# Clemapfel/egg_fluid_simulation

Measured on AMD Instinct MI355X. Metric: pair_solves_per_sec, higher is better.
Workload: dtype f64

## Files before the change

egg_fluid_simulation_amd/csrc/eggsim_device.h:

```cpp
#pragma once
#include <stdint.h>

#define EGG_MAX_PASSES 64
#define EGG_WAVE 64

struct EggStatus {
    int32_t fail_claim;
    int32_t fail_overflow;
    int32_t fail_stall;
    int32_t fail_range;
    int32_t min_slack;
    int32_t was_cut;
    int32_t fail_levels;
    int32_t max_level;
    int32_t fail_levlds;
    int32_t reserved0;
    unsigned long long visits[EGG_MAX_PASSES];
    unsigned long long max_list;
    unsigned long long rounds;
};

struct EggStepArgs {
    const double *x_in, *y_in, *vx_in, *vy_in;
    double *x_out, *y_out, *vx_out, *vy_out;
// ... 91 lines not shown
    double *pk_pos, *pk_prev, *pk_wr;
    int32_t *pk_src;
    int32_t *pk_atom;
    uint16_t *pk_aslot;
    uint32_t *pk_ckey;
    int32_t pk_stride;
    uint32_t *lists;
    uint16_t *lvl;
    uint32_t *rank;
    uint32_t *sorted;
    uint32_t *chunks;
    int32_t *grp_nchunks;
    uint32_t *lev_start;
    int32_t *grp_nlev;
    int32_t *tile_total;
    int32_t *tile_visits;
    int32_t *tile_need;
    int32_t *tile_slack;
    int32_t *tile_fast;
    int32_t lcap, scap, lev_cap, sort_cap, chunk_cap;
    int32_t nmax, amax, ccap, use_grid, stage_cap;
    double sub_delta, damping, follow_compliance, collision_compliance, overlap_factor, cell_size, eps;
    int32_t n_substeps, n_collision_steps;
    int32_t pass_seq, substep, stale;
    int32_t tune;
    uint32_t *simd_claims;
    int32_t lev_lds_cap;
    EggStatus *status, *status_next;
};
#define EGG_PK_MAX_PASSES 64
#define EGG_PK_WINDOW 128

static inline size_t egg_pk_lists_lds_bytes(int nmax, int amax, int ccap, int use_grid, int stage_cap, int gens) {
    size_t n = (size_t)nmax, a = (size_t)amax, c = (size_t)ccap, b = 0, G = (size_t)gens;
    b += egg_align16(G * n * 4);
    b += egg_align16(G * c * 4);
    b += egg_align16(use_grid ? 0 : G * c * 4);
    b += egg_align16((n + 1) * 4);
    b += egg_align16(n * 4);
    b += egg_align16(a * 4 * 4);
    b += egg_align16((a + 1) * 4);
    b += egg_align16(16 * 4);
    b += egg_align16(G * n * 2);
    b += egg_align16(n * 2);
    {
        const size_t stage = egg_align16(((size_t)stage_cap + 1) * (n + 1) * 2), tmp = egg_align16(n * 4) + egg_align16(n * 2);
        b += stage > tmp ? stage : tmp;
    }
    return b;
}
#define EGG_PK_SPIN_LIMIT (1u << 24)
#define EGG_PK_RING 8
#define EGG_PK_RING_BYTES (EGG_PK_RING * 64 * 56)
static inline size_t egg_pk_levels_mr_lds_bytes(int lev_cap, int group_particles, int threads) {
    return egg_align16((size_t)(lev_cap + 2) * 4) + egg_align16((size_t)group_particles * 2) +
           egg_align16((size_t)group_particles * 4) + egg_align16((size_t)(threads / 16) * EGG_PK_WINDOW * 4);
}
static inline size_t egg_pk_levels_ooo_lds_bytes(int lev_cap, int group_particles, int tiles, int lev_lds_cap) {
    return egg_align16((size_t)(lev_cap + 2) * 4) + egg_align16((size_t)group_particles * 4) + 2 * egg_align16((size_t)(group_particles + 64) * 4) +
           egg_align16((size_t)tiles * (size_t)lev_lds_cap * 2);
}

#define EGG_RENDER_TILE 16
#define EGG_RENDER_STAGE 128
struct EggRenderArgs {
    const double *x, *y, *last_x, *last_y, *vx, *vy, *radius;
    const int32_t *atom_offset;
    const float4 *atom_color;
    int32_t n, n_atoms;
    float t, tx, ty;
    float texture_scale, motion_blur;
    int32_t premultiply;
    int32_t cw, ch, tiles_x, tiles_y;
    uint32_t *tile_count, *tile_start, *tile_cursor;
    uint32_t *entries;
    uint32_t *totals;
    const float *texture;
    int32_t tsize;
    float4 *canvas;
};
static inline size_t egg_render_splat_lds_bytes(int tsize, size_t padded_list) {
    return egg_align16((size_t)(tsize + 2) * (tsize + 2) * 4) + (size_t)EGG_RENDER_STAGE * (32 + 16) + padded_list * 4;
}
struct EggCompositeLayer {
    const float4 *canvas;
    int32_t w, h;
    float x0, y0;
    float4 color, outline_color;
    float outline_thickness, highlight_strength, shadow_strength;
};
struct EggCompositeArgs {
    float4 *screen;
    int32_t screen_w, screen_h, n_layers;
    float threshold, smoothness;
    int32_t use_particle_color, use_lighting;
    EggCompositeLayer layer[2];
};

struct EggStepArgs4 {
    EggStepArgs a[4];
};

#define EGG_RX_EMPTY_KEY 0xFFFFFFFFFFFFFFFFull
struct EggRelaxedArgs {
    int32_t n;
    uint32_t table_mask;
// ... 153 lines not shown
```

egg_fluid_simulation_amd/csrc/eggsim_host_step.hip:

```cpp
#include "eggsim_host.h"

namespace egghost {


Env make_env(const egg_config &c, double sub_delta, int64_t n) {
    Env e;
    e.sub_delta = sub_delta;
    auto compliance = [&](double strength) {
        double alpha = 1 - clampd(strength, 0, 1);
        return alpha / (sub_delta * sub_delta);
    };
    e.damping = 1 - clampd(c.damping, 0, 1);
    e.follow_c = compliance(c.follow_strength);
    e.collision_c = compliance(c.collision_strength);
    e.cohesion_c = compliance(c.cohesion_strength);
    double nn = (double)n;
    e.budget = c.max_collision_fraction * (nn * nn);
    e.cell = cell_size_of(c);
    return e;
}

int launch_prologue(egg_handle *h, int which, hipStream_t stream) {
    System &s = h->sys[which];
    s.parity ^= 1;
// ... 136 lines not shown
    A.lvl = s.pk_lvl.p + pc.entry_base;
    A.rank = pc.levels_ooo ? s.pk_rank.p + pc.entry_base : nullptr;
    A.sorted = s.pk_sorted.p + pc.sort_base;
    A.chunks = s.pk_chunks.p + pc.chunk_base;
    A.grp_nchunks = s.pk_nchunks.p + pc.group_base;
    A.grp_nlev = s.pk_nchunks.p + s.pk_groups + pc.group_base;
    A.lev_start = s.pk_levstart.p + (size_t)pc.group_base * ((size_t)s.pk_lev_cap + 2);
    int32_t *tb = s.pk_tile.p + (size_t)pc.tile_base * (3 + 2 * EGG_PK_MAX_PASSES);
    A.tile_total = tb;
    A.tile_slack = tb + pc.n_tiles;
    A.tile_fast = tb + 2 * (size_t)pc.n_tiles;
    A.tile_visits = tb + 3 * (size_t)pc.n_tiles;
    A.tile_need = tb + (3 + (size_t)EGG_PK_MAX_PASSES) * (size_t)pc.n_tiles;
    A.lcap = pc.lcap;
    A.scap = pc.scap;
    A.lev_cap = s.pk_lev_cap;
    A.sort_cap = pc.sort_cap;
    A.chunk_cap = pc.chunk_cap;
    A.stage_cap = pc.stage_cap;
    A.nmax = lc.nmax;
    A.amax = lc.amax;
    A.ccap = lc.ccap;
    A.use_grid = lc.use_grid;
    A.sub_delta = env.sub_delta;
    A.damping = env.damping;
    A.follow_compliance = env.follow_c;
    A.collision_compliance = env.collision_c;
    A.overlap_factor = s.cfg.collision_overlap_factor;
    A.cell_size = env.cell;
    A.eps = s.cfg.eps;
    A.n_substeps = S;
    A.n_collision_steps = C;
    A.status = d_stat(s, s.parity);
    A.status_next = d_stat(s, s.parity ^ 1);
    A.tune = h->opt_tune;
    A.lev_lds_cap = pc.lev_lds_now;
    A.simd_claims = h->simd_claims.p;
}

int launch_packed(egg_handle *h, int which, const Env &env, int S, int C) {
    System &s = h->sys[which];
    const hipStream_t st = s.stream;
    if (s.pk_plan_dirty) {
        HIP_TRY(h, hipMemcpyAsync(s.pk_meta.p, s.pk_meta_host.data(), s.pk_meta_host.size() * sizeof(int32_t),
                                  hipMemcpyHostToDevice, st));
    }
    for (PackedClass &pc : s.pk) {
        if (!pc.levels_ooo) continue;
        int now = pc.lev_lds_cap;
        if (s.pk_seen_list) now = (int)std::min<size_t>((size_t)now, std::max<size_t>((size_t)(s.pk_seen_list + s.pk_seen_list / 4 + 256), s.pk_lev_lds_min));
        now = std::min(pc.lev_lds_cap, (now + 7) & ~7);
        pc.lev_lds_now = now;
        pc.lds_levels_now = egg_pk_levels_ooo_lds_bytes(s.pk_lev_cap, pc.max_group_particles, pc.max_tiles_in_group, now);
        pc.lds_pass_now = std::max(pc.lds_levels_now, pc.lds_exec + 64 * 16 + (size_t)EGG_PK_RING_BYTES);
    }
    std::vector<EggPackedArgs> args(s.pk.size());
    for (size_t k = 0; k < s.pk.size(); ++k) fill_packed_args(h, which, s.pk[k], env, S, C, args[k]);
    const bool stamp = h->opt_timing >= 2;
    s.pk_stamps_used = 0;
    auto stamp_begin = [&](int kind) -> System::PkStamp * {
        if (!stamp) return nullptr;
        if (s.pk_stamps_used == s.pk_stamps.size()) {
            System::PkStamp ps{nullptr, nullptr, 0, 0};
            if (hipEventCreate(&ps.a) != hipSuccess || hipEventCreate(&ps.b) != hipSuccess) return nullptr;
            s.pk_stamps.push_back(ps);
        }
        System::PkStamp *ps = &s.pk_stamps[s.pk_stamps_used++];
        ps->kind = kind;
        ps->launches = (int)s.pk.size();
        (void)hipEventRecord(ps->a, st);
        return ps;
    };
    auto launch_some = [&](int take, int kind, auto kernel_of, auto grid_of, auto block_of, auto lds_of) {
        System::PkStamp *ps = nullptr;
        for (size_t k = 0; k < s.pk.size(); ++k) {
            const PackedClass &pc = s.pk[k];
            if ((take == 1 && pc.fused_pass) || (take == 2 && !pc.fused_pass)) continue;
            if (!ps) ps = stamp_begin(kind);
            hipLaunchKernelGGL(kernel_of(pc), dim3((unsigned)grid_of(pc)), dim3((unsigned)block_of(pc)), lds_of(pc), st, args[k]);
            h->stats.kernel_launches++;
        }
        if (ps) (void)hipEventRecord(ps->b, st);
    };
    auto launch_all = [&](int kind, auto kernel_of, auto grid_of, auto block_of, auto lds_of) { launch_some(0, kind, kernel_of, grid_of, block_of, lds_of); };
    auto flat_grid = [](const PackedClass &pc) { return (pc.p_end - pc.p_begin + 255) / 256; };
    auto c256 = [](const PackedClass &) { return 256; };
    auto c64 = [](const PackedClass &) { return 64; };
    auto no_lds = [](const PackedClass &) { return (size_t)0; };
    auto tiles_of = [](const PackedClass &pc) { return pc.n_tiles; };
    auto groups_of = [](const PackedClass &pc) { return pc.n_groups; };
    if (s.pk_plan_dirty) {
        launch_all(-1, [](const PackedClass &) { return egg_pk_plan_kernel; }, tiles_of, c64, no_lds);
        s.pk_plan_dirty = false;
    }
    launch_all(EGG_PK_KIND_BEGIN, [](const PackedClass &) { return egg_pk_begin_kernel; }, flat_grid, c256, no_lds);
    int pass_seq = 0;
    for (int sub = 0; sub < S; ++sub) {
        if (sub > 0) launch_all(EGG_PK_KIND_MID, [](const PackedClass &) { return egg_pk_mid_kernel; }, flat_grid, c256, no_lds);
        for (int c = 0; c < C; ++c, ++pass_seq) {
            const bool stale = c == 0 && sub > 0;
            for (EggPackedArgs &A : args) {
                A.pass_seq = pass_seq;
                A.substep = sub;
                A.stale = stale ? 1 : 0;
            }
            launch_some(0, stale ? EGG_PK_KIND_LISTS_STALE : EGG_PK_KIND_LISTS_FRESH,
                        [&](const PackedClass &) { return stale ? egg_pk_lists_stale_kernel : egg_pk_lists_fresh_kernel; }, tiles_of,
// ... 460 lines not shown
```

egg_fluid_simulation_amd/csrc/eggsim_host_tiling.hip:

```cpp
#include "eggsim_host.h"

namespace egghost {




double g_retile_ms[8];
struct RetileLap {
    std::chrono::steady_clock::time_point t = std::chrono::steady_clock::now();
    void operator()(int k) {
        const auto n = std::chrono::steady_clock::now();
        g_retile_ms[k] += std::chrono::duration<double, std::milli>(n - t).count();
        t = n;
    }
};

int retile(egg_handle *h, int which) {
    System &s = h->sys[which];
    RetileLap lap;
    int rc = upload_atoms(h, which);
    if (rc != EGG_OK) return rc;
    const size_t na = s.atoms.size();
    const double cell = cell_size_of(s.cfg);
    s.extra_margin.resize(h->batches.size(), 0);
// ... 413 lines not shown
                                                     tiles[(size_t)lc.first_tile].particles);
            int max_tiles_in_group = 0;
            for (int t = 0; t < lc.n_tiles;) {
                int64_t in_group = 0;
                int t_end = t;
                while (t_end < lc.n_tiles && t_end - t < 64) {
                    const int64_t np = tiles[(size_t)lc.first_tile + t_end].particles;
                    if (t_end > t && (in_group + np > gp_max || in_group + np > 32767)) break;
                    in_group += np;
                    ++t_end;
                }
                const int32_t rec[4] = {t, t_end, tile_first_particle[(size_t)t], (int32_t)in_group};
                s.pk_meta_host.insert(s.pk_meta_host.end(), rec, rec + 4);
                pc.n_groups++;
                pc.max_group_particles = std::max<int>(pc.max_group_particles, (int)in_group);
                max_tiles_in_group = std::max(max_tiles_in_group, t_end - t);
                t = t_end;
            }
            const int simds = 4 * std::max(1, h->prop.multiProcessorCount);
            const bool dense_tiles = tiles[(size_t)lc.first_tile].particles > 256;
            pc.levels_ooo = h->lds_lane_ordered && h->opt_level_walk != 1 && (h->opt_level_walk == 2 || (pc.n_groups <= simds && dense_tiles));
            if (pc.levels_ooo) {
                const size_t guess = s.pk_seen_list ? (size_t)(s.pk_seen_list * 3 / 2 + 512) : (size_t)24 * lc.nmax;
                pc.lev_lds_cap = (int)std::min<size_t>((size_t)pc.scap, std::max<size_t>(guess, s.pk_lev_lds_min));
                pc.lev_lds_cap = (pc.lev_lds_cap + 7) & ~7;
                if (pc.n_groups > std::max(1, h->prop.multiProcessorCount)) {
                    const size_t budget = (kLdsMax - 4096) / 2;
                    const size_t fixed = egg_pk_levels_ooo_lds_bytes(s.pk_lev_cap, pc.max_group_particles, max_tiles_in_group, 0);
                    if (budget > fixed) {
                        const size_t fit = ((budget - fixed) / ((size_t)max_tiles_in_group * 2)) & ~(size_t)7;
                        const size_t need = std::max<size_t>((size_t)(s.pk_seen_list + s.pk_seen_list / 16 + 64), s.pk_lev_lds_min);
                        if (fit >= need && (size_t)pc.lev_lds_cap > fit) pc.lev_lds_cap = (int)fit;
                    }
                }
                pc.levels_threads = 64 * std::min(16, std::max(4, max_tiles_in_group <= 4 ? 2 * max_tiles_in_group : max_tiles_in_group));
                pc.lds_levels = egg_pk_levels_ooo_lds_bytes(s.pk_lev_cap, pc.max_group_particles, max_tiles_in_group, pc.lev_lds_cap);
                if (pc.lds_levels > h->lds_limit) pc.levels_ooo = 0;
            }
            pc.fused_pass = pc.levels_ooo && pc.levels_threads <= 512 && max_tiles_in_group <= 4 && pc.n_groups <= simds && !(h->opt_tune & 64);
            if (!pc.levels_ooo) {
                pc.levels_threads = std::min(256, (max_tiles_in_group * 16 + 63) / 64 * 64);
                pc.lds_levels = egg_pk_levels_mr_lds_bytes(s.pk_lev_cap, pc.max_group_particles, pc.levels_threads);
            }
            const size_t sort_words = (size_t)max_tiles_in_group * (size_t)pc.scap + 64;
            pc.chunk_cap = (int)std::min<size_t>(sort_words / 64 + (size_t)s.pk_lev_cap + 8, (size_t)1 << 28);
            pc.lds_exec = (size_t)pc.max_group_particles * 16;
            pc.lds_sort = egg_align16((size_t)(s.pk_lev_cap + 2) * 4) + sort_words * 4;
            if (pc.lds_sort > 64 * 1024) pc.lds_sort = 0;
            if (pc.lds_exec + 64 * 16 > h->lds_limit || pc.lds_levels > h->lds_limit || sort_words >= ((size_t)1 << 26)) {
                s.pk_meta_host.resize(meta_mark);
                continue;
            }
            if (pc.fused_pass) {
                pc.lds_pass = std::max(pc.lds_levels, pc.lds_exec + 64 * 16 + (size_t)EGG_PK_RING_BYTES);
                if (pc.lds_pass > h->lds_limit) pc.fused_pass = 0;
            }
            pc.sort_cap = (int)sort_words;
            pc.max_tiles_in_group = max_tiles_in_group;
            pc.lev_lds_now = pc.lev_lds_cap;
            pc.lds_levels_now = pc.lds_levels;
            pc.lds_pass_now = pc.lds_pass;
            if (getenv("EGGSIM_DEBUG"))
                fprintf(stderr, "eggsim: type %d packed class: %d tiles of <= %d particles in %d groups, grid cells %d (%s), lists: %d threads, %d staged partners, %zu B LDS; levels: %s, %d threads, %zu B LDS (level array %d entries); pass fused %d, %zu B LDS\n",
                        which, lc.n_tiles, lc.nmax, pc.n_groups, lc.ccap, lc.use_grid ? "dense grid" : "hash", pc.threads_lists, pc.stage_cap, pc.lds_lists,
                        pc.levels_ooo ? "out of order" : "in order", pc.levels_threads, pc.lds_levels, pc.lev_lds_cap, pc.fused_pass, pc.lds_pass);
            pc.chunk_base = s.pk_chunk_words;
            s.pk_chunk_words += (size_t)pc.n_groups * (size_t)pc.chunk_cap;
            lc.packed = (int)s.pk.size();
            s.pk_n = pn;
            s.pk_tiles += lc.n_tiles;
            s.pk_groups += pc.n_groups;
            s.pk_entries += (size_t)lc.n_tiles * (size_t)pc.scap;
            s.pk_sort_words += (size_t)pc.n_groups * (size_t)pc.sort_cap;
            s.pk.push_back(pc);
        }
        if (!s.pk.empty()) {
            s.pk_meta_claims = (s.pk_meta_host.size() + 3) & ~(size_t)3;
            s.pk_meta_host.resize(s.pk_meta_claims);
            for (int32_t a : s.tile_atoms) {
                const Box &c = claim[(size_t)a];
                const int32_t rec[4] = {c.lo_x, c.lo_y, c.hi_x, c.hi_y};
                s.pk_meta_host.insert(s.pk_meta_host.end(), rec, rec + 4);
            }
            lap(5);
            const size_t np = (size_t)s.pk_n, nt = (size_t)s.pk_tiles, ng = (size_t)s.pk_groups;
            HIP_TRY(h, s.pk_meta.reserve(s.pk_meta_host.size() + 4, false, s.stream));
            HIP_TRY(h, s.pk_src.reserve(np, false, s.stream));
            HIP_TRY(h, s.pk_atom.reserve(np, false, s.stream));
            HIP_TRY(h, s.pk_aslot.reserve(np + 8, false, s.stream));
            HIP_TRY(h, s.pk_pos.reserve(2 * np, false, s.stream));
            HIP_TRY(h, s.pk_prev.reserve(2 * np, false, s.stream));
            HIP_TRY(h, s.pk_wr.reserve(2 * np, false, s.stream));
            HIP_TRY(h, s.pk_ckey.reserve(2 * np, false, s.stream));
            HIP_TRY(h, s.pk_lists.reserve(s.pk_entries + 64, false, s.stream));
            HIP_TRY(h, s.pk_lvl.reserve(s.pk_entries + 64, false, s.stream));
            bool any_ooo = false;
            for (const PackedClass &pc : s.pk) any_ooo |= pc.levels_ooo != 0;
            if (any_ooo) HIP_TRY(h, s.pk_rank.reserve(s.pk_entries + 64, false, s.stream));
            HIP_TRY(h, s.pk_sorted.reserve(s.pk_sort_words + 64, false, s.stream));
            HIP_TRY(h, s.pk_chunks.reserve(s.pk_chunk_words + 64, false, s.stream));
            HIP_TRY(h, s.pk_nchunks.reserve(2 * ng + 8, false, s.stream));
            HIP_TRY(h, s.pk_levstart.reserve(ng * ((size_t)s.pk_lev_cap + 2) + 64, false, s.stream));
            HIP_TRY(h, s.pk_tile.reserve(nt * (3 + 2 * EGG_PK_MAX_PASSES) + 4, false, s.stream));
        }
        s.pk_plan_dirty = true;
    }

// ... 14 lines not shown
```

egg_fluid_simulation_amd/csrc/eggsim_packed.hip:

```cpp
#include <hip/hip_runtime.h>
#include "eggsim_device.h"

#include "eggsim_tile.h"

namespace {


__device__ inline uint32_t pk_cell_meta(const Tile &t, int gh, int buf, uint32_t key) {
    if (t.use_grid) return t.cell(buf)[(int)(key >> 16) * gh + (int)(key & 0xFFFFu)];
    return cell_meta(t, buf, key);
}

template <class F>
__device__ inline int pk_visit_fresh(const Tile &t, int gh, int cur, int i, F emit) {
    const uint32_t ki = t.ckey(cur)[i];
    const uint16_t *items = t.hitems(cur);
    int count = 0;
    if (t.use_grid) {
        const uint32_t *cells = t.cell(cur);
        const int h1 = (int)(ki >> 16) * gh + (int)(ki & 0xFFFFu);
#pragma unroll
        for (int p = 0; p < 3; ++p) {
            const int h0 = h1 + (p - 1) * gh - 1;
            const uint32_t m0 = cells[h0], m2 = cells[h0 + 2];
            const int st = (int)(m0 >> 16), en = (int)(m2 >> 16) + (int)(m2 & 0xFFFFu);
            for (int e = st; e < en; ++e) {
                const int j = items[e];
                if (j > i) {
                    emit(count, j);
                    ++count;
                }
            }
        }
        return count;
    }
    for (int p = 0; p < 3; ++p) {
        uint32_t m[3];
#pragma unroll
        for (int r = 0; r < 3; ++r) m[r] = cell_meta(t, cur, (uint32_t)((int)ki + (p - 1) * 65536 + (r - 1)));
#pragma unroll
        for (int r = 0; r < 3; ++r) {
            const int st = (int)(m[r] >> 16), cn = (int)(m[r] & 0xFFFFu);
            for (int e = 0; e < cn; ++e) {
                const int j = items[st + e];
                if (j > i) {
                    emit(count, j);
                    ++count;
                }
            }
        }
    }
    return count;
}
// ... 982 lines not shown
                    (flags >> 31) != 0, (flags & 0x8000u) != 0, pa, pb, wa[u].x, wb[u].x, (wa[u].x + wb[u].x) + compliance, pc[u], md2s[u], overlap,
                    compliance, eps);
                {
                    egg_v2d oa, ob;
                    oa.x = pa.x;
                    oa.y = pa.y;
                    ob.x = pb.x;
                    ob.y = pb.y;
                    *(store ? qa : spare) = oa;
                    *(store ? qb : spare) = ob;
                }
                __builtin_amdgcn_sched_barrier(0);
                qa = qa1;
                qb = qb1;
                flags = flags1;
            }
        }
#undef EGG_PIN
    } else {
        for (int c0 = 0; c0 < nch; c0 += R) {
#pragma unroll
            for (int u = 0; u < R; ++u) {
                const int c = c0 + u;
                rec[(u + D_REC) & (R - 1)] = load_rec(c + D_REC, dsc[(u + D_REC) & (R - 1)]);
                dsc[(u + D_DSC) & (R - 1)] = load_desc(c + D_DSC);
                wa[(u + D_WR) & (R - 1)] = gwr[rec[(u + D_WR) & (R - 1)] & 0x7FFFu];
                wb[(u + D_WR) & (R - 1)] = gwr[(rec[(u + D_WR) & (R - 1)] >> 16) & 0x7FFFu];
                pc[(u + D_PC) & (R - 1)] = pair_constants(wa[(u + D_PC) & (R - 1)], wb[(u + D_PC) & (R - 1)]);
                const uint32_t r0 = rec[u];
                if (r0 >> 31) {
                    const int ga = (int)(r0 & 0x7FFFu), gb = (int)((r0 >> 16) & 0x7FFFu);
                    double2 pa = lpos[ga], pb = lpos[gb];
                    project_pair<true>([&]() { return A.atom_batch[A.pk_atom[p0 + ga]] == A.atom_batch[A.pk_atom[p0 + gb]]; },
                                       (r0 & 0x8000u) != 0, pa, pb, wa[u], wb[u], pc[u], overlap, compliance, eps);
                    lpos[ga] = pa;
                    lpos[gb] = pb;
                }
            }
        }
    }
    for (int i = lane; i < np; i += 64) gpos[i] = lpos[i];
}
extern "C" __global__ void __launch_bounds__(64) egg_pk_exec_kernel(EggPackedArgs A) { egg_pk_exec_body<false>(A, blockIdx.x); }
extern "C" __global__ void __launch_bounds__(64) egg_pk_exec_chain_kernel(EggPackedArgs A) { egg_pk_exec_body<true>(A, blockIdx.x); }

typedef double egg_v2d __attribute__((ext_vector_type(2)));
typedef uint32_t egg_v2u __attribute__((ext_vector_type(2)));
typedef __attribute__((address_space(3))) egg_v2d egg_lds_v2d;
typedef __attribute__((address_space(3))) uint32_t egg_lds_u32;
struct PkRing {
    egg_v2d *a, *c, *d;
    egg_v2u *q;
    volatile egg_lds_u32 *produced, *consumed;
};
__device__ __forceinline__ PkRing pk_ring_at(unsigned char *base, uint32_t *produced, uint32_t *consumed) {
    PkRing r;
    r.a = (egg_v2d *)base;
    r.c = r.a + EGG_PK_RING * 64;
    r.d = r.c + EGG_PK_RING * 64;
    r.q = (egg_v2u *)(r.d + EGG_PK_RING * 64);
    r.produced = (volatile egg_lds_u32 *)produced;
    r.consumed = (volatile egg_lds_u32 *)consumed;
    return r;
}

__device__ __forceinline__ void egg_pk_exec_helper(const EggPackedArgs &A, const int g, const PkRing ring) {
    extern __shared__ __align__(16) unsigned char smem[];
    const int lane = threadIdx.x & 63;
    const int nch = A.grp_nchunks[g];
    if (nch <= 0) return;
    const int nch_pad = (nch + 7) & ~7;
    const int4 gg = ((const int4 *)A.grp_geo)[g];
    const int p0 = __builtin_amdgcn_readfirstlane(gg.z);
    egg_lds_v2d *const lp = (egg_lds_v2d *)smem;
    const double2 *gwr = (const double2 *)A.pk_wr + p0;
    const uint32_t *sorted = A.sorted + (size_t)g * A.sort_cap;
    typedef const __attribute__((address_space(4))) uint32_t egg_const_u32;
    egg_const_u32 *kchunks = (egg_const_u32 *)(uintptr_t)(A.chunks + (size_t)g * A.chunk_cap);
    const double overlap = A.overlap_factor, compliance = A.collision_compliance;
    auto load_desc = [&](int c) -> uint32_t { return kchunks[min(c, nch - 1)]; };
    auto load_rec = [&](int c, uint32_t desc) -> uint32_t {
        const uint32_t start = desc & 0x3FFFFFFu, cnt = (c < nch) ? (desc >> 26) + 1u : 0u;
        const uint32_t w = sorted[start + (uint32_t)lane];
        return ((uint32_t)lane < cnt) ? w : 0u;
    };
    constexpr int R = 8, D_DSC = 6, D_REC = 4, D_WR = 2;
    uint32_t dsc[R], rec[R];
    double2 wa[R], wb[R];
#pragma unroll
    for (int u = 0; u < D_DSC; ++u) dsc[u] = load_desc(u);
#pragma unroll
    for (int u = 0; u < D_REC; ++u) rec[u] = load_rec(u, dsc[u]);
#pragma unroll
    for (int u = 0; u < D_WR; ++u) {
        wa[u] = gwr[rec[u] & 0x7FFFu];
        wb[u] = gwr[(rec[u] >> 16) & 0x7FFFu];
    }
    int room = EGG_PK_RING;
    unsigned spins = 0;
    for (int k0 = 0; k0 < nch_pad; k0 += R) {
#pragma unroll
        for (int u = 0; u < R; ++u) {
            const int k = k0 + u;
            rec[(u + D_REC) & (R - 1)] = load_rec(k + D_REC, dsc[(u + D_REC) & (R - 1)]);
            dsc[(u + D_DSC) & (R - 1)] = load_desc(k + D_DSC);
            wa[(u + D_WR) & (R - 1)] = gwr[rec[(u + D_WR) & (R - 1)] & 0x7FFFu];
            wb[(u + D_WR) & (R - 1)] = gwr[(rec[(u + D_WR) & (R - 1)] >> 16) & 0x7FFFu];
            const uint32_t r0 = rec[u];
            const double2 a = wa[u], b = wb[u];
            egg_v2d ra, rc, rd;
            ra.x = a.x;
            ra.y = b.x;
            const double divisor = (a.x + b.x) + compliance;
            rc.x = egg_rcp_refined(divisor);
            rc.y = overlap * (a.y + b.y);
            rd.x = divisor;
            rd.y = rc.y * rc.y;
            egg_v2u rq;
            rq.x = (uint32_t)(uintptr_t)(lp + (r0 & 0x7FFFu)) | (r0 >> 31) | ((r0 >> 14) & 2u);
            rq.y = (uint32_t)(uintptr_t)(lp + ((r0 >> 16) & 0x7FFFu));
            if (k >= room) {
                for (;;) {
                    room = (int)__builtin_amdgcn_readfirstlane(*ring.consumed) + EGG_PK_RING;
                    if (k < room || ++spins >= EGG_PK_SPIN_LIMIT) break;
                    __builtin_amdgcn_s_sleep(1);
                }
            }
            const int slot = (u & (EGG_PK_RING - 1)) * 64 + lane;
            ring.a[slot] = ra;
            ring.c[slot] = rc;
            ring.d[slot] = rd;
            ring.q[slot] = rq;
            __asm__ volatile("" ::: "memory");
            *ring.produced = (uint32_t)(k + 1);
            __asm__ volatile("" ::: "memory");
        }
    }
    if (spins >= EGG_PK_SPIN_LIMIT && lane == 0) atomicExch(&A.status->fail_stall, 4);
}

__device__ __forceinline__ void egg_pk_exec_consumer(const EggPackedArgs &A, const int g, const PkRing ring) {
    extern __shared__ __align__(16) unsigned char smem[];
    const int lane = threadIdx.x & 63;
    const int nch = A.grp_nchunks[g];
    if (nch <= 0) return;
    const int nch_pad = (nch + 7) & ~7;
    const int4 gg = ((const int4 *)A.grp_geo)[g];
    const int p0 = __builtin_amdgcn_readfirstlane(gg.z), np = __builtin_amdgcn_readfirstlane(gg.w);
    double2 *lpos = (double2 *)smem;
    double2 *gpos = (double2 *)A.pk_pos + p0;
    for (int i0 = 0; i0 < np; i0 += 512) {
        double2 v[8];
#pragma unroll
        for (int u = 0; u < 8; ++u) v[u] = gpos[min(i0 + 64 * u + lane, np - 1)];
#pragma unroll
        for (int u = 0; u < 8; ++u) lpos[min(i0 + 64 * u + lane, np - 1)] = v[u];
    }
    const double overlap = A.overlap_factor, compliance = A.collision_compliance, eps = A.eps;
    egg_lds_v2d *const lp = (egg_lds_v2d *)smem;
    egg_lds_v2d *const spare = lp + np + lane;
    int seen = 0;
#ifdef EGG_PROFILE
    unsigned long long waited = 0, polls = 0;
#endif
    auto wait_for = [&](int chunk) {
        if (__builtin_expect(seen <= chunk, 0)) {
#ifdef EGG_PROFILE
            const unsigned long long w0 = __builtin_amdgcn_s_memtime();
            ++polls;
#endif
            for (unsigned spins = 0;; ++spins) {
                seen = (int)__builtin_amdgcn_readfirstlane(*ring.produced);
                if (seen > chunk) break;
                if (spins >= EGG_PK_SPIN_LIMIT) {
                    if (lane == 0) atomicExch(&A.status->fail_stall, 4);
                    seen = 0x7FFFFFFF;
                    break;
                }
                __builtin_amdgcn_s_sleep(1);
            }
#ifdef EGG_PROFILE
            waited += __builtin_amdgcn_s_memtime() - w0;
#endif
        }
        __asm__ volatile("" ::: "memory");
    };
    wait_for(0);
    egg_v2d ra = ring.a[lane], rc = ring.c[lane], rd = ring.d[lane];
    egg_v2u rq = ring.q[lane];
    uint32_t peek = 0;
    for (int c0 = 0; c0 < nch_pad; c0 += 8) {
#pragma unroll
        for (int u = 0; u < 8; ++u) {
            const int c = c0 + u;
            egg_lds_v2d *const qa = (egg_lds_v2d *)(uintptr_t)(rq.x & ~15u), *const qb = (egg_lds_v2d *)(uintptr_t)rq.y;
            const bool has_pair = (rq.x & 1u) != 0, slow = (rq.x & 2u) != 0;
            const egg_v2d va = *qa, vb = *qb;
            __builtin_amdgcn_sched_barrier(0);
            egg_v2d ra1 = ra, rc1 = rc, rd1 = rd;
            egg_v2u rq1 = rq;
            if (u < 7 || c + 1 < nch_pad) {
                seen = max(seen, (int)__builtin_amdgcn_readfirstlane(peek));
                wait_for(c + 1);
                peek = *ring.produced;
                const int slot = ((u + 1) & (EGG_PK_RING - 1)) * 64 + lane;
                ra1 = ring.a[slot];
                rc1 = ring.c[slot];
                rd1 = ring.d[slot];
                rq1 = ring.q[slot];
            }
            __builtin_amdgcn_sched_barrier(0);
            double2 pa = make_double2(va.x, va.y), pb = make_double2(vb.x, vb.y);
            const bool store = project_pair_predicated(
                [&]() { return A.atom_batch[A.pk_atom[p0 + (int)(qa - lp)]] == A.atom_batch[A.pk_atom[p0 + (int)(qb - lp)]]; }, []() {},
                [&](double2 &wra, double2 &wrb) {
                    wra = ((const double2 *)A.pk_wr)[p0 + (int)(qa - lp)];
                    wrb = ((const double2 *)A.pk_wr)[p0 + (int)(qb - lp)];
                },
                has_pair, slow, pa, pb, ra.x, ra.y, rd.x, make_double2(rc.x, rc.y), rd.y, overlap, compliance, eps);
            {
                egg_v2d oa, ob;
                oa.x = pa.x;
                oa.y = pa.y;
                ob.x = pb.x;
                ob.y = pb.y;
                *(store ? qa : spare) = oa;
                *(store ? qb : spare) = ob;
            }
            if (u == 3 || u == 7) {
                __asm__ volatile("" ::: "memory");
                *ring.consumed = (uint32_t)(c + 2);
            }
            __builtin_amdgcn_sched_barrier(0);
            ra = ra1;
            rc = rc1;
            rd = rd1;
            rq = rq1;
        }
    }
    for (int i = lane; i < np; i += 64) gpos[i] = lpos[i];
#ifdef EGG_PROFILE
    if (g == 0 && lane == 0) {
        A.status->visits[27] = waited;
        A.status->visits[26] = polls;
    }
#endif
}

extern "C" __global__ void __launch_bounds__(512) egg_pk_levexec_kernel(EggPackedArgs A) {
    extern __shared__ __align__(16) unsigned char smem[];
    const int g = blockIdx.x;
    if (g >= A.n_groups) return;
    pk_levels_ooo_body(A, g, (int)blockDim.x);
    __threadfence_block();
    __shared__ uint32_t simd_of_wave[8];
    __shared__ int exec_wave_s, help_wave_s;
    __shared__ uint32_t claim_key_s, claim_exec_s, claim_help_s;
    __shared__ uint32_t ring_produced, ring_consumed;
    const int wave = threadIdx.x >> 6;
    const uint32_t hw_id = __builtin_amdgcn_s_getreg(4 | (0 << 6) | (31 << 11));
    if ((threadIdx.x & 63) == 0) simd_of_wave[wave] = (hw_id >> 4) & 3u;
    __syncthreads();
    if (threadIdx.x == 0) {
        const uint32_t xcc = __builtin_amdgcn_s_getreg(20 | (0 << 6) | (3 << 11));
        const uint32_t key = ((hw_id >> 8) & 0xFFu) | (xcc << 8);
        const int nwaves = (int)(blockDim.x >> 6);
        uint32_t present = 0;
        for (int w = 0; w < nwaves; ++w) present |= 1u << simd_of_wave[w];
        uint32_t got[2] = {0, 0};
        uint32_t seen = __hip_atomic_load(&A.simd_claims[key], __ATOMIC_RELAXED, __HIP_MEMORY_SCOPE_AGENT);
        for (int role = 0; role < 2; ++role)
            for (int tries = 0; tries < 8; ++tries) {
                const uint32_t free_simds = present & ~seen & ~got[0] & 0xFu;
                if (!free_simds) break;
                const uint32_t want = free_simds & (0u - free_simds);
                const uint32_t prev = atomicOr(&A.simd_claims[key], want);
                seen = prev | want;
                if (!(prev & want)) {
                    got[role] = want;
                    break;
                }
            }
        int ew = -1, hw = -1;
        for (int w = 0; w < nwaves; ++w) {
            if (got[0] && ew < 0 && (1u << simd_of_wave[w]) == got[0]) ew = w;
            if (got[1] && hw < 0 && (1u << simd_of_wave[w]) == got[1]) hw = w;
        }
        if (ew < 0) ew = 0;
        if (hw < 0 || hw == ew) hw = (ew + 1) % nwaves;
        exec_wave_s = ew;
        help_wave_s = hw;
        claim_key_s = key;
        claim_exec_s = got[0];
        claim_help_s = got[1];
        ring_produced = 0;
        ring_consumed = 0;
    }
    __syncthreads();
    const int np = __builtin_amdgcn_readfirstlane(((const int4 *)A.grp_geo)[g].w);
    const PkRing ring = pk_ring_at(smem + egg_align16((size_t)(np + 64) * 16), &ring_produced, &ring_consumed);
    if (wave == help_wave_s) {
        __builtin_amdgcn_s_dcache_inv();
        egg_pk_exec_helper(A, g, ring);
        if ((threadIdx.x & 63) == 0 && claim_help_s) atomicAnd(&A.simd_claims[claim_key_s], ~claim_help_s);
        return;
    }
    if (wave != exec_wave_s) return;
    EGG_STAMP(E0);
#ifdef EGG_PROFILE
    const unsigned long long R0 = __builtin_amdgcn_s_memrealtime();
#endif
    __builtin_amdgcn_s_setprio(3);
    egg_pk_exec_consumer(A, g, ring);
    if ((threadIdx.x & 63) == 0 && claim_exec_s) atomicAnd(&A.simd_claims[claim_key_s], ~claim_exec_s);
#ifdef EGG_PROFILE
    __asm__ volatile("s_waitcnt vmcnt(0) lgkmcnt(0)" ::: "memory");
    EGG_STAMP(E1);
    if ((threadIdx.x & 63) == 0) {
        const unsigned long long nch = (unsigned long long)max(A.grp_nchunks[g], 1);
        if (g == 0) {
            A.status->visits[30] = E1 - E0;
            A.status->visits[31] = nch;
            A.status->visits[28] = __builtin_amdgcn_s_memrealtime() - R0;
        }
        atomicMax(&A.status->visits[32], (E1 - E0) * 16ull / nch);
        const uint32_t simd = (hw_id >> 4) & 3u;
        if (simd < 3) atomicAdd(&A.status->visits[33 + simd], 1ull);
        if (!claim_exec_s) atomicAdd(&A.status->visits[29], 1ull);
    }
#endif
}

extern "C" __global__ void __launch_bounds__(256) egg_pk_end_kernel(EggPackedArgs A) {
    const int tile = blockIdx.x;
    if (tile >= A.n_tiles) return;
    const int tid = threadIdx.x, nthreads = blockDim.x;
    const int4 geo = ((const int4 *)A.tile_geo)[2 * tile];
    const int a_begin = geo.z, na = geo.w;
    __shared__ int32_t red[8];
    __shared__ int32_t wslack[4];
    int slack = 0x7FFFFFFF;
    int p = geo.x;
    for (int k = 0; k < na; ++k) {
        const int atom = A.tile_atoms[a_begin + k];
        const int cnt = A.atom_count[atom];
        __syncthreads();
        if (tid < 8) red[tid] = (tid < 2) ? 0x7FFFFFFF : (tid < 4) ? -0x7FFFFFFF : 0;
        __syncthreads();
        const int4 clv = ((const int4 *)A.tile_claims)[a_begin + k];
        const int32_t cl[4] = {clv.x, clv.y, clv.z, clv.w};
        int lo_x = 0x7FFFFFFF, lo_y = 0x7FFFFFFF, hi_x = -0x7FFFFFFF, hi_y = -0x7FFFFFFF;
        int d0 = 0, d1 = 0, d2 = 0, d3 = 0;
        for (int q = tid; q < cnt; q += nthreads) {
// ... 107 lines not shown
```

Baseline: 10.98 billion.

## Forward particle positions across chunks and deepen consumer ring prefetch

The helper wave now assigns each pair to a ring lane so that a particle reused in the next chunk stays on the same lane. The consumer can then forward the updated position in a register instead of re-reading LDS. The helper also flags chunks that have no read-after-write hazard, so the consumer can load the next chunk's positions early, and the ring prefetch distance grows from one chunk to two. This targets the LDS load latency on the serial dependency chain, at the cost of extra LDS bookkeeping (lane_of, written, taken, freelist), more helper work and a larger LDS footprint.

New measurement: 6.938 billion. 0.632x the previous value.

```diff
diff --git a/egg_fluid_simulation_amd/csrc/eggsim_device.h b/egg_fluid_simulation_amd/csrc/eggsim_device.h
--- a/egg_fluid_simulation_amd/csrc/eggsim_device.h
+++ b/egg_fluid_simulation_amd/csrc/eggsim_device.h
@@ -167,6 +167,7 @@
 #define EGG_PK_SPIN_LIMIT (1u << 24)
 #define EGG_PK_RING 8
 #define EGG_PK_RING_BYTES (EGG_PK_RING * 64 * 56)
+#define EGG_PK_FWD_BYTES(group_particles) (2 * egg_align16((size_t)((group_particles) + 64) * 4) + 2 * 128 * 4)
 static inline size_t egg_pk_levels_mr_lds_bytes(int lev_cap, int group_particles, int threads) {
     return egg_align16((size_t)(lev_cap + 2) * 4) + egg_align16((size_t)group_particles * 2) +
            egg_align16((size_t)group_particles * 4) + egg_align16((size_t)(threads / 16) * EGG_PK_WINDOW * 4);
diff --git a/egg_fluid_simulation_amd/csrc/eggsim_host_step.hip b/egg_fluid_simulation_amd/csrc/eggsim_host_step.hip
--- a/egg_fluid_simulation_amd/csrc/eggsim_host_step.hip
+++ b/egg_fluid_simulation_amd/csrc/eggsim_host_step.hip
@@ -212,7 +212,7 @@
         now = std::min(pc.lev_lds_cap, (now + 7) & ~7);
         pc.lev_lds_now = now;
         pc.lds_levels_now = egg_pk_levels_ooo_lds_bytes(s.pk_lev_cap, pc.max_group_particles, pc.max_tiles_in_group, now);
-        pc.lds_pass_now = std::max(pc.lds_levels_now, pc.lds_exec + 64 * 16 + (size_t)EGG_PK_RING_BYTES);
+        pc.lds_pass_now = std::max(pc.lds_levels_now, pc.lds_exec + 64 * 16 + (size_t)EGG_PK_RING_BYTES + EGG_PK_FWD_BYTES(pc.max_group_particles));
     }
     std::vector<EggPackedArgs> args(s.pk.size());
     for (size_t k = 0; k < s.pk.size(); ++k) fill_packed_args(h, which, s.pk[k], env, S, C, args[k]);
diff --git a/egg_fluid_simulation_amd/csrc/eggsim_host_tiling.hip b/egg_fluid_simulation_amd/csrc/eggsim_host_tiling.hip
--- a/egg_fluid_simulation_amd/csrc/eggsim_host_tiling.hip
+++ b/egg_fluid_simulation_amd/csrc/eggsim_host_tiling.hip
@@ -489,7 +489,7 @@
                 continue;
             }
             if (pc.fused_pass) {
-                pc.lds_pass = std::max(pc.lds_levels, pc.lds_exec + 64 * 16 + (size_t)EGG_PK_RING_BYTES);
+                pc.lds_pass = std::max(pc.lds_levels, pc.lds_exec + 64 * 16 + (size_t)EGG_PK_RING_BYTES + EGG_PK_FWD_BYTES(pc.max_group_particles));
                 if (pc.lds_pass > h->lds_limit) pc.fused_pass = 0;
             }
             pc.sort_cap = (int)sort_words;
diff --git a/egg_fluid_simulation_amd/csrc/eggsim_packed.hip b/egg_fluid_simulation_amd/csrc/eggsim_packed.hip
--- a/egg_fluid_simulation_amd/csrc/eggsim_packed.hip
+++ b/egg_fluid_simulation_amd/csrc/eggsim_packed.hip
@@ -1,4 +1,5 @@
 #include <hip/hip_runtime.h>
+#include <type_traits>
 #include "eggsim_device.h"
 
 #include "eggsim_tile.h"
@@ -1087,13 +1088,18 @@
     egg_v2d *a, *c, *d;
     egg_v2u *q;
     volatile egg_lds_u32 *produced, *consumed;
+    egg_lds_u32 *lane_of, *written, *taken, *freelist;
 };
-__device__ __forceinline__ PkRing pk_ring_at(unsigned char *base, uint32_t *produced, uint32_t *consumed) {
+__device__ __forceinline__ PkRing pk_ring_at(unsigned char *base, uint32_t *produced, uint32_t *consumed, int np) {
     PkRing r;
     r.a = (egg_v2d *)base;
     r.c = r.a + EGG_PK_RING * 64;
     r.d = r.c + EGG_PK_RING * 64;
     r.q = (egg_v2u *)(r.d + EGG_PK_RING * 64);
+    r.lane_of = (egg_lds_u32 *)(base + EGG_PK_RING_BYTES);
+    r.written = r.lane_of + egg_align16((size_t)(np + 64) * 4) / 4;
+    r.taken = r.written + egg_align16((size_t)(np + 64) * 4) / 4;
+    r.freelist = r.taken + 128;
     r.produced = (volatile egg_lds_u32 *)produced;
     r.consumed = (volatile egg_lds_u32 *)consumed;
     return r;
@@ -1106,13 +1112,18 @@
     if (nch <= 0) return;
     const int nch_pad = (nch + 7) & ~7;
     const int4 gg = ((const int4 *)A.grp_geo)[g];
-    const int p0 = __builtin_amdgcn_readfirstlane(gg.z);
+    const int p0 = __builtin_amdgcn_readfirstlane(gg.z), np = __builtin_amdgcn_readfirstlane(gg.w);
     egg_lds_v2d *const lp = (egg_lds_v2d *)smem;
     const double2 *gwr = (const double2 *)A.pk_wr + p0;
     const uint32_t *sorted = A.sorted + (size_t)g * A.sort_cap;
     typedef const __attribute__((address_space(4))) uint32_t egg_const_u32;
     egg_const_u32 *kchunks = (egg_const_u32 *)(uintptr_t)(A.chunks + (size_t)g * A.chunk_cap);
     const double overlap = A.overlap_factor, compliance = A.collision_compliance;
+    for (int i = lane; i < np + 64; i += 64) {
+        ring.lane_of[i] = 0u;
+        ring.written[i] = 0u;
+    }
+    ring.taken[lane] = 0u;
     auto load_desc = [&](int c) -> uint32_t { return kchunks[min(c, nch - 1)]; };
     auto load_rec = [&](int c, uint32_t desc) -> uint32_t {
         const uint32_t start = desc & 0x3FFFFFFu, cnt = (c < nch) ? (desc >> 26) + 1u : 0u;
@@ -1151,9 +1162,25 @@
             rc.y = overlap * (a.y + b.y);
             rd.x = divisor;
             rd.y = rc.y * rc.y;
+            const uint32_t ia = r0 & 0x7FFFu, ib = (r0 >> 16) & 0x7FFFu;
+            const bool hp = (r0 >> 31) != 0;
+            const uint32_t lo = ring.lane_of[ia], wra = ring.written[ia], wrb = ring.written[ib];
+            const bool inherit = hp && (lo >> 6) == (uint32_t)(k + 1);
+            ring.taken[inherit ? (lo & 63u) : 64u + (uint32_t)lane] = (uint32_t)(k + 1);
+            const bool unsafe = hp && (wrb == (uint32_t)(k + 1) || (!inherit && wra == (uint32_t)(k + 1)));
+            const uint64_t free_lanes = __ballot(ring.taken[lane] != (uint32_t)(k + 1));
+            const uint32_t free_rank = __builtin_amdgcn_mbcnt_hi((uint32_t)(free_lanes >> 32), __builtin_amdgcn_mbcnt_lo((uint32_t)free_lanes, 0u));
+            ring.freelist[((free_lanes >> lane) & 1ull) ? free_rank : 64u + (uint32_t)lane] = (uint32_t)lane;
+            const uint64_t fresh = ~__ballot(inherit);
+            const uint32_t fresh_rank = __builtin_amdgcn_mbcnt_hi((uint32_t)(fresh >> 32), __builtin_amdgcn_mbcnt_lo((uint32_t)fresh, 0u));
+            const uint32_t target = inherit ? (lo & 63u) : ring.freelist[fresh_rank];
+            const uint32_t early_safe = __ballot(unsafe) == 0ull ? 8u : 0u;
+            ring.lane_of[hp ? ia : (uint32_t)(np + lane)] = ((uint32_t)(k + 2) << 6) | target;
+            ring.written[hp ? ia : (uint32_t)(np + lane)] = (uint32_t)(k + 2);
+            ring.written[hp ? ib : (uint32_t)(np + lane)] = (uint32_t)(k + 2);
             egg_v2u rq;
-            rq.x = (uint32_t)(uintptr_t)(lp + (r0 & 0x7FFFu)) | (r0 >> 31) | ((r0 >> 14) & 2u);
-            rq.y = (uint32_t)(uintptr_t)(lp + ((r0 >> 16) & 0x7FFFu));
+            rq.x = (uint32_t)(uintptr_t)(lp + ia) | (r0 >> 31) | ((r0 >> 14) & 2u) | (inherit ? 4u : 0u) | early_safe;
+            rq.y = (uint32_t)(uintptr_t)(lp + ib);
             if (k >= room) {
                 for (;;) {
                     room = (int)__builtin_amdgcn_readfirstlane(*ring.consumed) + EGG_PK_RING;
@@ -1161,7 +1188,7 @@
                     __builtin_amdgcn_s_sleep(1);
                 }
             }
-            const int slot = (u & (EGG_PK_RING - 1)) * 64 + lane;
+            const int slot = (u & (EGG_PK_RING - 1)) * 64 + (int)target;
             ring.a[slot] = ra;
             ring.c[slot] = rc;
             ring.d[slot] = rd;
@@ -1198,79 +1225,105 @@
 #ifdef EGG_PROFILE
     unsigned long long waited = 0, polls = 0;
 #endif
-    auto wait_for = [&](int chunk) {
-        if (__builtin_expect(seen <= chunk, 0)) {
+    auto wait_slow = [&](int chunk) -> bool {
+        bool gone = false;
 #ifdef EGG_PROFILE
-            const unsigned long long w0 = __builtin_amdgcn_s_memtime();
-            ++polls;
+        const unsigned long long w0 = __builtin_amdgcn_s_memtime();
+        ++polls;
 #endif
-            for (unsigned spins = 0;; ++spins) {
-                seen = (int)__builtin_amdgcn_readfirstlane(*ring.produced);
-                if (seen > chunk) break;
-                if (spins >= EGG_PK_SPIN_LIMIT) {
-                    if (lane == 0) atomicExch(&A.status->fail_stall, 4);
-                    seen = 0x7FFFFFFF;
-                    break;
-                }
-                __builtin_amdgcn_s_sleep(1);
-            }
+        for (unsigned spins = 0;; ++spins) {
+            seen = (int)__builtin_amdgcn_readfirstlane(*ring.produced);
+            if (seen > chunk) break;
+            if (spins >= EGG_PK_SPIN_LIMIT) {
+                if (lane == 0) atomicExch(&A.status->fail_stall, 4);
+                gone = true;
+                break;
+            }
+            __builtin_amdgcn_s_sleep(1);
+        }
 #ifdef EGG_PROFILE
-            waited += __builtin_amdgcn_s_memtime() - w0;
+        waited += __builtin_amdgcn_s_memtime() - w0;
 #endif
-        }
-        __asm__ volatile("" ::: "memory");
+        return gone;
     };
-    wait_for(0);
+    bool gone = false;
+    if (wait_slow(1)) gone = true;
     egg_v2d ra = ring.a[lane], rc = ring.c[lane], rd = ring.d[lane];
     egg_v2u rq = ring.q[lane];
+    egg_v2d ra1 = ring.a[64 + lane], rc1 = ring.c[64 + lane], rd1 = ring.d[64 + lane];
+    egg_v2u rq1 = ring.q[64 + lane];
+    egg_v2d va = *lp, vb = *lp, carry = *lp;
+    bool pre = false;
     uint32_t peek = 0;
-    for (int c0 = 0; c0 < nch_pad; c0 += 8) {
+    auto turn = [&](auto early_tag, const int u, const int c) -> bool {
+        constexpr bool EARLY = decltype(early_tag)::value;
+        egg_lds_v2d *const qa = (egg_lds_v2d *)(uintptr_t)(rq.x & ~15u), *const qb = (egg_lds_v2d *)(uintptr_t)rq.y;
+        const bool has_pair = (rq.x & 1u) != 0, slow = (rq.x & 2u) != 0, forwarded = (rq.x & 4u) != 0;
+        if (!pre) {
+            va = *qa;
+            vb = *qb;
+        }
+        egg_v2d va1 = va, vb1 = vb;
+        if (EARLY) {
+            va1 = *(egg_lds_v2d *)(uintptr_t)(rq1.x & ~15u);
+            vb1 = *(egg_lds_v2d *)(uintptr_t)rq1.y;
+        }
+        __builtin_amdgcn_sched_barrier(0);
+        egg_v2d ra2 = ra1, rc2 = rc1, rd2 = rd1;
+        egg_v2u rq2 = rq1;
+        if (u < 6 || c + 2 < nch_pad) {
+            seen = max(seen, (int)__builtin_amdgcn_readfirstlane(peek));
+            if (__builtin_expect(seen <= c + 2, 0) && wait_slow(c + 2)) return true;
+            __asm__ volatile("" ::: "memory");
+            peek = *ring.produced;
+            const int slot = ((u + 2) & (EGG_PK_RING - 1)) * 64 + lane;
+            ra2 = ring.a[slot];
+            rc2 = ring.c[slot];
+            rd2 = ring.d[slot];
+            rq2 = ring.q[slot];
+        }
+        __builtin_amdgcn_sched_barrier(0);
+        double2 pa = make_double2(forwarded ? carry.x : va.x, forwarded ? carry.y : va.y), pb = make_double2(vb.x, vb.y);
+        const double2 pa_in = pa;
+        const bool store = project_pair_predicated(
+            [&]() { return A.atom_batch[A.pk_atom[p0 + (int)(qa - lp)]] == A.atom_batch[A.pk_atom[p0 + (int)(qb - lp)]]; }, []() {},
+            [&](double2 &wra, double2 &wrb) {
+                wra = ((const double2 *)A.pk_wr)[p0 + (int)(qa - lp)];
+                wrb = ((const double2 *)A.pk_wr)[p0 + (int)(qb - lp)];
+            },
+            has_pair, slow, pa, pb, ra.x, ra.y, rd.x, make_double2(rc.x, rc.y), rd.y, overlap, compliance, eps);
+        {
+            egg_v2d oa, ob;
+            oa.x = pa.x;
+            oa.y = pa.y;
+            ob.x = pb.x;
+            ob.y = pb.y;
+            *(store ? qa : spare) = oa;
+            *(store ? qb : spare) = ob;
+            carry.x = store ? pa.x : pa_in.x;
+            carry.y = store ? pa.y : pa_in.y;
+        }
+        if (u == 3 || u == 7) {
+            __asm__ volatile("" ::: "memory");
+            *ring.consumed = (uint32_t)(c + 3);
+        }
+        __builtin_amdgcn_sched_barrier(0);
+        ra = ra1, rc = rc1, rd = rd1, rq = rq1;
+        ra1 = ra2, rc1 = rc2, rd1 = rd2, rq1 = rq2;
+        va = va1;
+        vb = vb1;
+        pre = EARLY;
+        return false;
+    };
+    for (int c0 = 0; c0 < nch_pad && !gone; c0 += 8) {
 #pragma unroll
         for (int u = 0; u < 8; ++u) {
-            const int c = c0 + u;
-            egg_lds_v2d *const qa = (egg_lds_v2d *)(uintptr_t)(rq.x & ~15u), *const qb = (egg_lds_v2d *)(uintptr_t)rq.y;
-            const bool has_pair = (rq.x & 1u) != 0, slow = (rq.x & 2u) != 0;
-            const egg_v2d va = *qa, vb = *qb;
-            __builtin_amdgcn_sched_barrier(0);
-            egg_v2d ra1 = ra, rc1 = rc, rd1 = rd;
-            egg_v2u rq1 = rq;
-            if (u < 7 || c + 1 < nch_pad) {
-                seen = max(seen, (int)__builtin_amdgcn_readfirstlane(peek));
-                wait_for(c + 1);
-                peek = *ring.produced;
-                const int slot = ((u + 1) & (EGG_PK_RING - 1)) * 64 + lane;
-                ra1 = ring.a[slot];
-                rc1 = ring.c[slot];
-                rd1 = ring.d[slot];
-                rq1 = ring.q[slot];
-            }
-            __builtin_amdgcn_sched_barrier(0);
-            double2 pa = make_double2(va.x, va.y), pb = make_double2(vb.x, vb.y);
-            const bool store = project_pair_predicated(
-                [&]() { return A.atom_batch[A.pk_atom[p0 + (int)(qa - lp)]] == A.atom_batch[A.pk_atom[p0 + (int)(qb - lp)]]; }, []() {},
-                [&](double2 &wra, double2 &wrb) {
-                    wra = ((const double2 *)A.pk_wr)[p0 + (int)(qa - lp)];
-                    wrb = ((const double2 *)A.pk_wr)[p0 + (int)(qb - lp)];
-                },
-                has_pair, slow, pa, pb, ra.x, ra.y, rd.x, make_double2(rc.x, rc.y), rd.y, overlap, compliance, eps);
-            {
-                egg_v2d oa, ob;
-                oa.x = pa.x;
-                oa.y = pa.y;
-                ob.x = pb.x;
-                ob.y = pb.y;
-                *(store ? qa : spare) = oa;
-                *(store ? qb : spare) = ob;
-            }
-            if (u == 3 || u == 7) {
-                __asm__ volatile("" ::: "memory");
-                *ring.consumed = (uint32_t)(c + 2);
-            }
-            __builtin_amdgcn_sched_barrier(0);
-            ra = ra1;
-            rc = rc1;
-            rd = rd1;
-            rq = rq1;
+            const bool last = u == 7 && c0 + 8 >= nch_pad;
+            const bool early = !last && (__builtin_amdgcn_readfirstlane(rq1.x) & 8u) != 0;
+            if (early ? turn(std::true_type{}, u, c0 + u) : turn(std::false_type{}, u, c0 + u)) {
+                gone = true;
+                break;
+            }
         }
     }
     for (int i = lane; i < np; i += 64) gpos[i] = lpos[i];
@@ -1333,7 +1386,7 @@
     }
     __syncthreads();
     const int np = __builtin_amdgcn_readfirstlane(((const int4 *)A.grp_geo)[g].w);
-    const PkRing ring = pk_ring_at(smem + egg_align16((size_t)(np + 64) * 16), &ring_produced, &ring_consumed);
+    const PkRing ring = pk_ring_at(smem + egg_align16((size_t)(np + 64) * 16), &ring_produced, &ring_consumed, np);
     if (wave == help_wave_s) {
         __builtin_amdgcn_s_dcache_inv();
         egg_pk_exec_helper(A, g, ring);
```
